# uuwee/Vulkan-PBR-Renderer

Hardware: AMD Instinct MI355X
Metric: IBL-prefilter Mtexels/s (specular prefilter all mips + irradiance; PBR-shaded Mpixels/s under extra.shade_c5 / extra.shade) (higher is better)
Workload: dtype f32; 1 GPU; C4: 4096x4096 specular prefilter (6 faces, 13 mips) + 128x128 irradiance from a 2048^2 HDR cube; env=procedural HDR cube 2048^2 x6 RGBA32F (seed 0x5eed0004, RGBE round-tripped), overlap=False, parallelism=single GPU

## Files before the change

include/gpux.h:

```cpp
#ifndef GPUX_H
#define GPUX_H

#include "gpu_hip.h"

GPU_API void GPUX_SetDevice(int hip_device_index);
GPU_API int  GPUX_GetDevice(void);
typedef void (*GPUX_ErrorHandler)(const char* message, void* user);
GPU_API void GPUX_SetErrorHandler(GPUX_ErrorHandler handler, void* user);
GPU_API const char* GPUX_BackendName(void);

typedef struct GPUX_IBLConstants {
    int32_t mip_level;
    float   roughness;
    float   src_lod;
    int32_t sample_count;
} GPUX_IBLConstants;

GPU_API void GPUX_OpDispatchRows(GPU_Graph* graph, uint32_t face0, uint32_t face1, uint32_t row0, uint32_t row1);
GPU_API void GPUX_OpDispatchLines(GPU_Graph* graph, uint32_t y0, uint32_t y1, uint32_t z0, uint32_t z1);

enum { GPUX_Shade_IBL = 1 << 0, GPUX_Shade_LightShafts = 1 << 1,
       GPUX_Shade_SunShadows = 1 << 2,
       GPUX_Shade_VoxelGI = 1 << 3      };
GPU_API void GPUX_SetShadeFlags(GPU_GraphicsPipeline* pipeline, int flags);
GPU_API void GPUX_OpDrawRows(GPU_Graph* graph, uint32_t row0, uint32_t row1);

GPU_API void GPUX_OpCopyTextureMipToBuffer(GPU_Graph* graph, GPU_Texture* src, uint32_t mip_level, GPU_Buffer* dst, uint32_t dst_offset);
GPU_API void GPUX_OpCopyBufferToTextureMip(GPU_Graph* graph, GPU_Buffer* src, uint32_t src_offset, GPU_Texture* dst, uint32_t mip_level);
GPU_API uint64_t GPUX_TextureMipBytes(const GPU_Texture* texture, uint32_t mip_level);
GPU_API void GPUX_OpCopyDecodedTextureMipToBuffer(GPU_Graph* graph, GPU_Texture* src, uint32_t mip_level, GPU_Buffer* dst, uint32_t dst_offset);
GPU_API void GPUX_OpProjectSH9(GPU_Graph* graph, GPU_Texture* cube, uint32_t mip_level, uint32_t face0, uint32_t face1, uint32_t row0, uint32_t row1,
                               GPU_Buffer* dst, uint32_t dst_offset);
GPU_API void GPUX_OpIrradianceFromSH9(GPU_Graph* graph, GPU_Buffer* src, uint32_t src_offset, GPU_Texture* irradiance_cube, uint32_t mip_level);
GPU_API void* GPUX_TextureDevicePtr(GPU_Texture* texture, uint32_t mip_level);
GPU_API void* GPUX_BufferDevicePtr(GPU_Buffer* buffer);
GPU_API void* GPUX_GraphStream(GPU_Graph* graph);

GPU_API GPU_Texture* GPUX_MakeTextureExternal(GPU_Format format, uint32_t width, uint32_t height, uint32_t depth, GPU_TextureFlags flags,
                                              void* device_memory, uint64_t device_bytes);
GPU_API void GPUX_InvalidateTexture(GPU_Texture* texture);
GPU_API uint64_t GPUX_TextureTotalBytes(const GPU_Texture* texture);
GPU_API uint64_t GPUX_TextureMipOffset(const GPU_Texture* texture, uint32_t mip_level);

GPU_API GPU_Texture* GPUX_MakeCubemapFromEquirect(const void* rgba32f, uint32_t width, uint32_t height, uint32_t face_size, GPU_TextureFlags extra_flags);

GPU_API void GPUX_EnableOpTiming(int enable);
GPU_API uint32_t GPUX_GraphTimedOpCount(GPU_Graph* graph);
GPU_API const char* GPUX_GraphTimedOpName(GPU_Graph* graph, uint32_t index);
GPU_API float GPUX_GraphTimedOpMs(GPU_Graph* graph, uint32_t index);
GPU_API void GPUX_SetPrefilterTolerance(float rel);
GPU_API int GPUX_PrefilterKeptSamples(uint32_t mip_level);
GPU_API float GPUX_GraphSpanMs(GPU_Graph* graph);

GPU_API void GPUX_SetTileStreams(int count);

GPU_API void GPUX_SetGraphReplay(int enable);
GPU_API void GPUX_GraphReplayStats(GPU_Graph* graph, uint64_t* launches, uint64_t* updates, uint64_t* instantiations);
GPU_API uint64_t GPUX_FoldedBlitCount(void);
GPU_API void GPUX_SetGraphOverlap(int on);
GPU_API uint64_t GPUX_OverlappedSubmitCount(void);

GPU_API uint64_t GPUX_RasterRejectedTriangles(void);
GPU_API uint64_t GPUX_VoxelizeFragments(void);

#endif
```

vulkan-pbr-renderer_amd/csrc/gpu_hip.cpp:

```cpp
#include <hip/hip_runtime.h>

#include <math.h>
#include <stdarg.h>
#include <stdio.h>
#include <stdlib.h>
#include <string.h>

#include <map>
#include <string>
#include <vector>

#include "gpux.h"
#include "pbr_kernels.h"

static GPUX_ErrorHandler g_err_handler = nullptr;
static void* g_err_user = nullptr;

static void gpu_fail(const char* fmt, ...) {
    char buf[1024];
    va_list ap;
    va_start(ap, fmt);
    vsnprintf(buf, sizeof buf, fmt, ap);
    va_end(ap);
    if (g_err_handler) { g_err_handler(buf, g_err_user); return; }
    fprintf(stderr, "GPU-ERROR: %s\n", buf);
    fflush(stderr);
    abort();
}
#define GPU_REQUIRE(cond, ret, ...) do { if (!(cond)) { gpu_fail(__VA_ARGS__); return ret; } } while (0)
#define GPU_REQUIRE_V(cond, ...) do { if (!(cond)) { gpu_fail(__VA_ARGS__); return; } } while (0)
#define HIP_OK(call) do { hipError_t e_ = (call); if (e_ != hipSuccess) { gpu_fail("%s: HIP call failed: %s (%s)", __func__, #call, hipGetErrorString(e_)); } } while (0)

enum BindKind { Bind_Texture, Bind_Sampler, Bind_Buffer, Bind_StorageImage };
enum KernelId { Kernel_None = 0, Kernel_BrdfLut, Kernel_Irradiance, Kernel_Prefilter, Kernel_Lighting, Kernel_LightgridSweep, Kernel_TaaResolve, Kernel_FinalPost, Kernel_BloomDown, Kernel_BloomUp, Kernel_SunDepth, Kernel_Geometry, Kernel_Voxelize };

static bool is_bloom_kernel(KernelId k) { return k == Kernel_BloomDown || k == Kernel_BloomUp; }
static bool is_post_kernel(KernelId k) { return is_bloom_kernel(k) || k == Kernel_FinalPost || k == Kernel_TaaResolve; }

struct GPU_Sampler { GPU_SamplerDesc desc; bool shared; };

struct LayoutBinding { std::string name; BindKind kind; GPU_Format format; };
struct GPU_PipelineLayout { std::vector<LayoutBinding> bindings; bool finalized = false; };

struct TextureImpl {
    GPU_Texture base;
    void* dev = nullptr;
    size_t bytes = 0;
    std::vector<size_t> mip_offset;
    uint32_t texel_bytes = 0;
    void* bordered = nullptr;
    size_t bordered_bytes = 0;
    bool bordered_valid = false;
    int bordered_from = 0;
    bool owns_memory = true;
    void* decoded = nullptr; std::vector<size_t> decoded_offset;
    void* cells = nullptr; int cells_first = 0; std::vector<size_t> cells_off; std::vector<char> cells_valid;
    void* lut_cells = nullptr; bool lut_cells_valid = false;
    std::vector<char> range_valid; std::vector<float> range_min, range_max; void* range_dev = nullptr;
};
struct BufferImpl {
// ... 50 lines not shown
    hipEvent_t mid_ev = nullptr;
    bool mid_recorded = false;
    std::vector<TextureImpl*> tail_reads, tail_writes;
    size_t sync_used = 0;
    std::vector<Op> ops;
    bool submitted = false;
    GPU_ComputePipeline* bound_cpipe = nullptr;
    GPU_DescriptorSet* bound_cset = nullptr;
    uint8_t push[128]; uint32_t push_size = 0;
    GPU_RenderPass* preparing = nullptr; GPU_RenderPass* in_pass = nullptr;
    std::vector<DrawParams> draw_params;
    int bound_draw = -1;
    BufferImpl* vertex_buffer = nullptr; BufferImpl* index_buffer = nullptr;
    int raster_op = -1;
    std::vector<RasterScratch> raster; size_t raster_used = 0;
    void* sh_scratch = nullptr; size_t sh_scratch_bytes = 0;
    hipGraphExec_t exec = nullptr;
    bool replay_broken = false;
    uint64_t replay_launches = 0, replay_updates = 0, replay_instantiations = 0;
    std::vector<uint8_t> launch_sig, exec_sig;
    std::vector<hipEvent_t> ev;
    std::vector<std::string> timed_names;
    std::vector<float> timed_ms;
    hipEvent_t span_a = nullptr, span_b = nullptr;
    bool span_recorded = false;
    float span_ms = 0.0f;
};

struct DeviceTable { void* dev = nullptr; int count = 0; float alpha = 0.0f; std::vector<float> weights;  };
struct TableKey {
    int kind, n, aux; uint32_t rbits;
    bool operator<(const TableKey& o) const {
        if (kind != o.kind) return kind < o.kind;
        if (n != o.n) return n < o.n;
        if (aux != o.aux) return aux < o.aux;
        return rbits < o.rbits;
    }
};

static struct {
    GPU_Graph* last_submitted = nullptr;
    bool init = false;
    int device = -1;
    GPU_Sampler samplers[6];
    std::map<TableKey, DeviceTable> tables;
    bool timing = false;
    float prefilter_tol = 0.0f;
    int kept_samples[32] = {0};
    int fold = -1;
    int order = -1;
    int overlap = -1;
    int replay = -1;
    int tile_streams = -1;
    unsigned long long* raster_rejected = nullptr;
    uint64_t raster_rejected_base = 0;
} G;

static const char kTokenLut[] = "HIPK1:gen_brdf_integration_map";
static const char kTokenIrr[] = "HIPK3:gen_irradiance_map";
static const char kTokenPre[] = "HIPK4:gen_prefiltered_env_map";
static const char kTokenLit[] = "HIPK5:lighting_pass";
static const char kTokenSweep[] = "HIPK7:lightgrid_sweep";
static const char kTokenTaa[] = "HIPK8:taa_resolve";
static const char kTokenFinal[] = "HIPK9:final_post_process";
static const char kTokenBloomDown[] = "HIPK10:bloom_downsample";
static const char kTokenBloomUp[] = "HIPK11:bloom_upsample";
static const char kTokenSun[] = "HIPK12:sun_depth_pass";
static const char kTokenGeometry[] = "HIPK13:geometry_pass";
static const char kTokenVoxelize[] = "HIPK14:lightgrid_voxelize";

GPU_API GPU_FormatInfo GPUX_GetFormatInfo(GPU_Format f) {
    struct Row { GPU_Format f; uint32_t ext, size; bool s, v, c, d, st, i; const char* glsl; };
    static const Row rows[] = {
        {GPU_Format_R8UN, 1, 1, 1, 1, 1, 0, 0, 0, "r8"}, {GPU_Format_RG8UN, 1, 2, 1, 1, 1, 0, 0, 0, "rg8"},
        {GPU_Format_RGBA8UN, 1, 4, 1, 1, 1, 0, 0, 0, "rgba8"}, {GPU_Format_BGRA8UN, 1, 4, 1, 1, 1, 0, 0, 0, nullptr},
        {GPU_Format_R16F, 1, 2, 1, 1, 1, 0, 0, 0, "r16f"}, {GPU_Format_RG16F, 1, 4, 1, 1, 1, 0, 0, 0, "rg16f"},
        {GPU_Format_RGB16F, 1, 6, 0, 1, 0, 0, 0, 0, nullptr}, {GPU_Format_RGBA16F, 1, 8, 1, 1, 1, 0, 0, 0, "rgba16f"},
        {GPU_Format_R32F, 1, 4, 1, 1, 1, 0, 0, 0, "r32f"}, {GPU_Format_RG32F, 1, 8, 1, 1, 1, 0, 0, 0, "rg32f"},
        {GPU_Format_RGB32F, 1, 12, 0, 1, 0, 0, 0, 0, nullptr}, {GPU_Format_RGBA32F, 1, 16, 1, 1, 1, 0, 0, 0, "rgba32f"},
        {GPU_Format_R8I, 1, 1, 1, 1, 1, 0, 0, 1, "r8ui"}, {GPU_Format_R16I, 1, 2, 1, 1, 1, 0, 0, 1, "r16ui"},
        {GPU_Format_RG16I, 1, 4, 1, 1, 1, 0, 0, 1, "rg16ui"}, {GPU_Format_RGBA16I, 1, 8, 1, 1, 1, 0, 0, 1, "rgba16ui"},
        {GPU_Format_R32I, 1, 4, 1, 1, 1, 0, 0, 1, "r32ui"}, {GPU_Format_RG32I, 1, 8, 1, 1, 1, 0, 0, 1, "rg32ui"},
        {GPU_Format_RGB32I, 1, 12, 1, 1, 0, 0, 0, 1, nullptr}, {GPU_Format_RGBA32I, 1, 16, 1, 1, 1, 0, 0, 1, "rgba32ui"},
        {GPU_Format_R64I, 1, 8, 0, 0, 0, 0, 0, 1, "r64ui"}, {GPU_Format_D16UN, 1, 2, 1, 0, 0, 1, 0, 0, nullptr},
        {GPU_Format_D32F_Or_X8D24UN, 1, 4, 1, 0, 0, 1, 0, 0, nullptr}, {GPU_Format_D32FS8I_Or_D24UNS8I, 1, 5, 0, 0, 0, 1, 0, 0, nullptr},
        {GPU_Format_D24UNS8I_Or_D32FS8I, 1, 4, 0, 0, 0, 1, 0, 0, nullptr},
        {GPU_Format_BC1_RGB_UN, 4, 8, 1, 0, 0, 0, 0, 0, nullptr}, {GPU_Format_BC1_RGBA_UN, 4, 8, 1, 0, 0, 0, 0, 0, nullptr},
        {GPU_Format_BC3_RGBA_UN, 4, 16, 1, 0, 0, 0, 0, 0, nullptr}, {GPU_Format_BC5_UN, 4, 16, 1, 0, 0, 0, 0, 0, nullptr},
    };
    for (const Row& r : rows)
        if (r.f == f) { GPU_FormatInfo o = {r.ext, r.size, r.s, r.v, r.c, r.d, r.st, r.i, r.glsl}; return o; }
    GPU_FormatInfo z = {0, 0, false, false, false, false, false, false, nullptr};
    return z;
}

GPU_API void GPUX_SetDevice(int idx) { G.device = idx; }
GPU_API int GPUX_GetDevice(void) { return G.device; }
GPU_API void GPUX_SetErrorHandler(GPUX_ErrorHandler h, void* user) { g_err_handler = h; g_err_user = user; }
GPU_API const char* GPUX_BackendName(void) { return "hip-gfx950"; }

static void make_shared_sampler(GPU_Sampler* s, GPU_Filter f, GPU_AddressMode m) {
    memset(&s->desc, 0, sizeof s->desc);
    s->desc.min_filter = s->desc.mag_filter = s->desc.mipmap_mode = f;
    s->desc.address_modes[0] = s->desc.address_modes[1] = s->desc.address_modes[2] = m;
    s->desc.max_lod = 1000.0f;
    s->shared = true;
}

GPU_API void GPU_Init(GPU_WindowHandle window) {
    (void)window;
// ... 1472 lines not shown
    const bool explicit_c = ibl_constants(op, c);
    int n = (explicit_c && c.sample_count > 0) ? c.sample_count : 4096;
    DeviceTable* ang = get_table(2, n, 0.0f, 0);
    DeviceTable* vcs = get_table(3, (int)size, 0.0f, 0);
    if (!ang || !vcs) return;
    int fmt = ot->base.format == GPU_Format_RG16F ? PBRK_FMT_RG16F : (ot->base.format == GPU_Format_RG32F ? PBRK_FMT_RG32F : PBRK_FMT_RGBA32F);
    timed(g, "K1.brdf_lut", ev_used, [&] {
        int rc = pbrk_brdf_lut(out_ptr, fmt, (int)size, n, ang->dev, vcs->dev, (int)op.row0, (int)op.row1, g->cur);
        if (rc != PBRK_OK) gpu_fail("K1 launch failed (%d)", rc);
    });
    ot->bordered_valid = false; ot->lut_cells_valid = false;
}

struct IblPlan {
    bool ok = true;
    bool bad_roughness = false;
    bool copy = false;
    int mip = 0;
    float lod = 0.0f;
    int n = 0;
    float rough = 0.0f, divisor = 1.0f;
    int table_kind = -1;
    DeviceTable* tab = nullptr;
    char name[96];
};
static IblPlan plan_ibl(const Op& op) {
    IblPlan p;
    GPUX_IBLConstants c;
    const bool explicit_c = ibl_constants(op, c);
    p.mip = c.mip_level;
    if (op.cpipe->kernel == Kernel_Irradiance) {
        p.lod = explicit_c ? c.src_lod : 6.0f;
        p.n = (explicit_c && c.sample_count > 0) ? c.sample_count : 1024;
        p.divisor = (float)p.n; p.table_kind = 1;
        snprintf(p.name, sizeof p.name, "K3.irradiance");
    } else if (p.mip == 0) {
        p.copy = true; p.lod = explicit_c ? c.src_lod : 1.0f;
        snprintf(p.name, sizeof p.name, "K4a.prefilter_copy.mip%d", p.mip);
    } else {
        p.lod = explicit_c ? c.src_lod : 3.0f + (float)p.mip;
        p.n = (explicit_c && c.sample_count > 0) ? c.sample_count : 8192;
        p.rough = explicit_c ? c.roughness : reference_roughness(p.mip);
        p.divisor = 3.14159265358979323846f; p.table_kind = 0;
        snprintf(p.name, sizeof p.name, "K4b.prefilter_mc.mip%d", p.mip);
        if (!(p.rough > 0.0f)) { p.bad_roughness = true; p.ok = false; return p; }
    }
    if (p.table_kind >= 0) {
        p.tab = get_table(p.table_kind, p.n, p.rough, 0);
        p.ok = p.tab != nullptr;
    }
    return p;
}

static void exec_ibl_filter(GPU_Graph* g, Op& op, size_t& ev_used) {
    hipStream_t st = g->cur;
    Slot* out = named_slot(op.set, "OUTPUT");
    TextureImpl* ot = out->tex;
    uint32_t size = mip_dim(ot->base.width, out->mip);
    void* out_ptr = (char*)ot->dev + ot->mip_offset[out->mip];
    TextureImpl* et = named_slot(op.set, "TEX_ENV_CUBE")->tex;
    int W = (int)et->base.width, levels = (int)et->base.mip_level_count;
    const IblPlan p = plan_ibl(op);
    if (p.bad_roughness) { gpu_fail("prefilter: roughness must be > 0 for Monte-Carlo mips (got %g)", p.rough); return; }
    if (!p.ok) return;
    const bool mc_prefilter = op.cpipe->kernel == Kernel_Prefilter && !p.copy;
    int l = (int)floorf(p.lod);
    if (l < 0) l = 0;
    if (l > levels - 1) l = levels - 1;
    if ((float)l != p.lod && p.lod < (float)(levels - 1)) { gpu_fail("%s: fractional source LOD %g is not supported by the precompute kernels", p.name, p.lod); return; }
    if (!et->bordered_valid || et->bordered_from > l) {
        timed(g, "apron.env", ev_used, [&] { ensure_bordered(et, st, l); });
        if (!et->bordered_valid || et->bordered_from > l) return;
        publish_side_work(g);
    }
    int n_src = W >> l; if (n_src < 1) n_src = 1;
    const void* src = (const char*)et->bordered + pbrk_bordered_level_offset(W, l) * 16;
    const void* cells = nullptr;
    if (!p.copy) {
        if (cells_ready(et, l)) cells = ensure_cells(et, l, st);
        else { timed(g, "cells.env", ev_used, [&] { cells = ensure_cells(et, l, st); }); publish_side_work(g); }
    }
    int n_keep = p.tab ? p.tab->count : 0;
    if (mc_prefilter && G.prefilter_tol > 0.0f) {
        float mn = 0.0f, mx = 0.0f;
        if (level_range(et, l, st, &mn, &mx)) n_keep = bounded_sample_count(p.tab, mn, mx, G.prefilter_tol);
    }
    if (mc_prefilter && p.mip >= 0 && p.mip < 32) G.kept_samples[p.mip] = n_keep;
    const float alpha = p.table_kind == 0 ? p.tab->alpha : 0.0f;
    timed(g, p.name, ev_used, [&] {
        int rc = p.copy ? pbrk_prefilter_copy(src, n_src, out_ptr, (int)size, (int)op.face0, (int)op.face1, (int)op.row0, (int)op.row1, st)
                        : pbrk_mc_filter(src, cells, n_src, p.tab->dev, n_keep, p.divisor, alpha, out_ptr, (int)size,
                                         (int)op.face0, (int)op.face1, (int)op.row0, (int)op.row1, st);
        if (rc != PBRK_OK) gpu_fail("%s launch failed (%d)", p.name, rc);
    });
    ot->bordered_valid = false;
}

static double dispatch_samples_per_texel(const Op& op) {
    const IblPlan p = plan_ibl(op);
    if (op.cpipe->kernel == Kernel_Irradiance) return p.n;
    if (p.copy) return 4.0;
    return p.tab ? (double)p.tab->count : (double)p.n;
}

static void exec_bloom(GPU_Graph* g, Op& op, size_t& ev_used) {
    GPU_RenderPass* rp = op.pass;
    TextureImpl* target = (TextureImpl*)rp->targets[0].texture;
    TextureImpl* in = named_slot(op.set, "TEX0")->tex;
    PbrkBloomArgs a;
    a.src.data = (char*)in->dev + in->mip_offset[op.mip]; a.src.format = PBRK_FMT_RGBA16F;
    a.src.width = (int)mip_dim(in->base.width, op.mip); a.src.height = (int)mip_dim(in->base.height, op.mip);
    a.dst = (char*)target->dev + target->mip_offset[op.mip2];
    a.dst_width = (int)rp->desc.width; a.dst_height = (int)rp->desc.height;
    int32_t lvl; memcpy(&lvl, op.push, 4); a.dst_mip_level = lvl;
    a.upsample = op.gpipe->kernel == Kernel_BloomUp; a.blend_additive = op.gpipe->blend_additive;
    a.blend_src = op.blend_tex ? (const void*)((const char*)op.blend_tex->dev + op.blend_tex->mip_offset[op.blend_mip]) : nullptr;
    a.y0 = (int)op.row0; a.y1 = (int)op.row1;
    timed(g, a.upsample ? "K11.bloom_upsample" : "K10.bloom_downsample", ev_used, [&] {
        int rc = pbrk_bloom_pass(&a, g->cur);
        if (rc != PBRK_OK) gpu_fail("bloom launch failed (%d)", rc);
    });
}

static void exec_taa(GPU_Graph* g, Op& op, size_t& ev_used) {
    GPU_DescriptorSet* s = op.set;
    GPU_RenderPass* rp = op.pass;
    TextureImpl* target = (TextureImpl*)rp->targets[0].texture;
    PbrkTaaArgs a;
    a.lighting_result = tex2d(named_slot(s, "LIGHTING_RESULT")->tex, PBRK_FMT_RGBA16F);
    a.gbuffer_depth = tex2d(named_slot(s, "GBUFFER_DEPTH")->tex, PBRK_FMT_R32F);
    a.gbuffer_velocity = tex2d(named_slot(s, "GBUFFER_VELOCITY")->tex, PBRK_FMT_RG16F);
    a.gbuffer_velocity_prev = tex2d(named_slot(s, "GBUFFER_VELOCITY_PREV")->tex, PBRK_FMT_RG16F);
    a.prev_frame_result = tex2d(named_slot(s, "PREV_FRAME_RESULT")->tex, PBRK_FMT_RGBA16F);
    a.out = target->dev; a.out_format = out_fmt(target->base.format);
    a.width = (int)rp->desc.width; a.height = (int)rp->desc.height; a.y0 = (int)op.row0; a.y1 = (int)op.row1;
    timed(g, "K8.taa_resolve", ev_used, [&] {
        int rc = pbrk_taa_resolve(&a, g->cur);
        if (rc != PBRK_OK) gpu_fail("K8 launch failed (%d)", rc);
    });
}

static void exec_final(GPU_Graph* g, Op& op, size_t& ev_used) {
    GPU_RenderPass* rp = op.pass;
    TextureImpl* target = (TextureImpl*)rp->targets[0].texture;
    PbrkFinalArgs a;
    a.src = tex2d(named_slot(op.set, "TEX0")->tex, PBRK_FMT_RGBA16F);
    a.out = target->dev; a.out_format = out_fmt(target->base.format);
    a.width = (int)rp->desc.width; a.height = (int)rp->desc.height; a.y0 = (int)op.row0; a.y1 = (int)op.row1;
    timed(g, "K9.final_post_process", ev_used, [&] {
        int rc = pbrk_final_post_process(&a, g->cur);
        if (rc != PBRK_OK) gpu_fail("K9 launch failed (%d)", rc);
    });
}

static void exec_gridview(GPU_Graph* g, Op& op, size_t& ev_used, const float* globals) {
// ... 371 lines not shown
        return true;
    case Op_MipGen: r.push_back(op.tex); w.push_back(op.tex); return true;
    case Op_Blit: r.push_back(op.tex); w.push_back(op.tex2); return true;
    case Op_Clear: w.push_back(op.tex); return true;
    case Op_ProjectSH9: r.push_back(op.tex); return false;
    case Op_IrradianceSH9: w.push_back(op.tex); return false;
    default: return false;
    }
}
static uint64_t g_overlapped_submits = 0;
GPU_API void GPUX_SetGraphOverlap(int on) { G.overlap = on; }
GPU_API uint64_t GPUX_OverlappedSubmitCount(void) { return g_overlapped_submits; }
static bool contains(const std::vector<TextureImpl*>& v, const TextureImpl* t) { for (const TextureImpl* x : v) if (x == t) return true; return false; }

struct OrderPoint {
    GPU_Graph* prev = nullptr;
    size_t before = 0;
};
static OrderPoint order_after_previous(GPU_Graph* g) {
    OrderPoint o;
    GPU_Graph* prev = G.last_submitted;
    G.last_submitted = g;
    if (!env_setting(G.order, "PBR_GRAPH_ORDER", 1) || !prev || prev == g) return o;
    if (!prev->order_ev) HIP_OK(hipEventCreateWithFlags(&prev->order_ev, hipEventDisableTiming));
    HIP_OK(hipEventRecord(prev->order_ev, prev->stream));
    if (overlap_enabled() && prev->mid_recorded && !replay_enabled()) {
        std::vector<TextureImpl*> r, w;
        for (; o.before < g->ops.size(); ++o.before) {
            r.clear(); w.clear();
            if (!op_access(g->ops[o.before], r, w)) break;
            bool clash = false;
            for (TextureImpl* t : w) clash |= contains(prev->tail_reads, t) || contains(prev->tail_writes, t);
            for (TextureImpl* t : r) clash |= contains(prev->tail_writes, t);
            if (clash) break;
        }
    }
    if (o.before > 0) { HIP_OK(hipStreamWaitEvent(g->stream, prev->mid_ev, 0)); o.prev = prev; ++g_overlapped_submits; }
    else HIP_OK(hipStreamWaitEvent(g->stream, prev->order_ev, 0));
    return o;
}

static size_t split_head_tail(GPU_Graph* g, bool overlap_on) {
    size_t mid_idx = g->ops.size();
    for (size_t i = 0; i < g->ops.size(); ++i)
        if (g->ops[i].kind == Op_Shade && is_bloom_kernel(g->ops[i].gpipe->kernel)) { mid_idx = i; break; }
    g->mid_recorded = false; g->tail_reads.clear(); g->tail_writes.clear();
    if (!overlap_on || mid_idx == 0) return g->ops.size();
    bool known = true;
    for (size_t i = mid_idx; i < g->ops.size() && known; ++i) known = op_access(g->ops[i], g->tail_reads, g->tail_writes);
    if (!known) { mid_idx = g->ops.size(); g->tail_reads.clear(); g->tail_writes.clear(); }
    return mid_idx;
}

struct TileRegion {
    struct Wr { TextureImpl* t; uint32_t mip, f0, f1, r0, r1; };
    GPU_Graph* g;
    int n_side;
    std::vector<Wr> writes; std::vector<TextureImpl*> reads;
    bool open = false; size_t rr = 0;

    explicit TileRegion(GPU_Graph* graph) : g(graph) {
        env_setting(G.tile_streams, "PBR_TILE_STREAMS", 4);
        if (G.tile_streams > 16) G.tile_streams = 16;
        n_side = G.tile_streams;
    }
    void close() {
        if (!open) return;
        for (hipStream_t s : g->side) { hipEvent_t e = next_sync_event(g); HIP_OK(hipEventRecord(e, s)); HIP_OK(hipStreamWaitEvent(g->stream, e, 0)); }
        writes.clear(); reads.clear(); open = false; g->cur = g->stream;
    }
    bool wants_side_stream(const Op& op, Slot*& out, Slot*& env) const {
        out = env = nullptr;
        if (!(n_side >= 2 && op.kind == Op_Dispatch && op.rows_explicit && (op.cpipe->kernel == Kernel_Prefilter || op.cpipe->kernel == Kernel_Irradiance))) return false;
        out = named_slot(op.set, "OUTPUT");
        env = named_slot(op.set, "TEX_ENV_CUBE");
        bool tile = true;
        if (out && out->tex) {
            uint32_t size = mip_dim(out->tex->base.width, out->mip);
            double evals = (double)(op.face1 - op.face0) * (op.row1 - op.row0) * size * dispatch_samples_per_texel(op);
            bool whole = op.face0 == 0 && op.face1 == out->tex->base.layer_count && op.row0 == 0 && op.row1 == size;
            if (evals >= (whole ? 1.0e9 : 2.0e6 * 8192.0)) tile = false;
            if (whole && !open) tile = false;
        }
        return tile && out && env && out->tex && env->tex;
    }
    bool place(const Op& op) {
        Slot* out; Slot* env;
        if (!wants_side_stream(op, out, env)) { close(); return false; }
        Wr w = {out->tex, out->mip, op.face0, op.face1, op.row0, op.row1};
        bool clash = w.t == env->tex;
        for (const Wr& o : writes) {
            if (o.t == env->tex) clash = true;
            if (o.t == w.t && o.mip == w.mip && o.f0 < w.f1 && w.f0 < o.f1 && o.r0 < w.r1 && w.r0 < o.r1) clash = true;
        }
        for (TextureImpl* r : reads) if (r == w.t) clash = true;
        if (clash) close();
        if (w.t == env->tex) return false;
        if (!open) {
            while ((int)g->side.size() > n_side) { (void)hipStreamSynchronize(g->side.back()); (void)hipStreamDestroy(g->side.back()); g->side.pop_back(); }
            while ((int)g->side.size() < n_side) { hipStream_t s; HIP_OK(hipStreamCreateWithFlags(&s, hipStreamNonBlocking)); g->side.push_back(s); }
            hipEvent_t e = next_sync_event(g);
            HIP_OK(hipEventRecord(e, g->stream));
            for (hipStream_t s : g->side) HIP_OK(hipStreamWaitEvent(s, e, 0));
            open = true;
        }
        writes.push_back(w); reads.push_back(env->tex);
        g->cur = g->side[rr++ % g->side.size()];
        return true;
    }
};

static bool begin_capture(GPU_Graph* g) {
    if (!replay_enabled() || G.timing || g->replay_broken || g->ops.empty() || !graph_replayable(g)) return false;
    if (hipStreamBeginCapture(g->stream, hipStreamCaptureModeRelaxed) == hipSuccess) return true;
    (void)hipGetLastError(); g->replay_broken = true;
    return false;
}
static void finish_capture(GPU_Graph* g, size_t& ev_used) {
    hipGraph_t cg = nullptr;
    bool ok = hipStreamEndCapture(g->stream, &cg) == hipSuccess && cg;
    if (g->exec && g->exec_sig != g->launch_sig) { (void)hipGraphExecDestroy(g->exec); g->exec = nullptr; }
    if (ok && g->exec) {
        hipGraphNode_t bad = nullptr; hipGraphExecUpdateResult res;
        if (hipGraphExecUpdate(g->exec, cg, &bad, &res) == hipSuccess) ++g->replay_updates;
        else { (void)hipGetLastError(); (void)hipGraphExecDestroy(g->exec); g->exec = nullptr; }
    }
    if (ok && !g->exec) {
        if (hipGraphInstantiate(&g->exec, cg, nullptr, nullptr, 0) == hipSuccess) { ++g->replay_instantiations; g->exec_sig = g->launch_sig; }
        else { (void)hipGetLastError(); g->exec = nullptr; ok = false; }
    }
    if (ok && hipGraphLaunch(g->exec, g->stream) == hipSuccess) ++g->replay_launches; else ok = false;
    if (cg) (void)hipGraphDestroy(cg);
    if (ok) return;
    (void)hipGetLastError();
    g->replay_broken = true;
    if (g->exec) { (void)hipGraphExecDestroy(g->exec); g->exec = nullptr; }
    for (Op& op : g->ops) exec_op(g, op, ev_used);
}

GPU_API void GPU_GraphSubmit(GPU_Graph* g) {
    GPU_REQUIRE_V(g && !g->submitted, "GPU_GraphSubmit: graph is NULL or already submitted");
    GPU_REQUIRE_V(g->in_pass == nullptr && g->preparing == nullptr, "GPU_GraphSubmit: render pass still open");
    if (!snapshot_raster_draws(g)) return;
    g->timed_names.clear(); g->timed_ms.clear();
    size_t ev_used = 0;
    g->sync_used = 0;
    g->launch_sig.clear();
    g->cur = g->stream;
    fold_blits(g);
    OrderPoint order = order_after_previous(g);
    const size_t mid_idx = split_head_tail(g, overlap_enabled());
    if (order.before > mid_idx) order.before = mid_idx;
    g->span_recorded = false;
    if (G.timing) {
        if (!g->span_a) { HIP_OK(hipEventCreate(&g->span_a)); HIP_OK(hipEventCreate(&g->span_b)); }
        HIP_OK(hipEventRecord(g->span_a, g->stream));
    }
    const bool capture = begin_capture(g);
    TileRegion region(g);
    for (size_t i = 0; i < g->ops.size(); ++i) {
        if (order.prev && i == order.before) {
            region.close();
            HIP_OK(hipStreamWaitEvent(g->stream, order.prev->order_ev, 0));
            order.prev = nullptr;
        }
        if (i == mid_idx && !capture) {
            region.close();
            if (!g->mid_ev) HIP_OK(hipEventCreateWithFlags(&g->mid_ev, hipEventDisableTiming));
            HIP_OK(hipEventRecord(g->mid_ev, g->stream));
            g->mid_recorded = true;
        }
        region.place(g->ops[i]);
        exec_op(g, g->ops[i], ev_used);
        g->cur = g->stream;
    }
    region.close();
    if (order.prev) HIP_OK(hipStreamWaitEvent(g->stream, order.prev->order_ev, 0));
    if (G.timing) { HIP_OK(hipEventRecord(g->span_b, g->stream)); g->span_recorded = true; }
    if (capture) finish_capture(g, ev_used);
    g->submitted = true;
}

GPU_API void GPU_GraphWait(GPU_Graph* g) {
    GPU_REQUIRE_V(g, "GPU_GraphWait: NULL graph");
    HIP_OK(hipStreamSynchronize(g->stream));
    g->timed_ms.clear();
    for (size_t i = 0; i < g->timed_names.size(); ++i) {
        float ms = 0.0f;
        HIP_OK(hipEventElapsedTime(&ms, g->ev[2 * i], g->ev[2 * i + 1]));
        g->timed_ms.push_back(ms);
    }
    g->span_ms = 0.0f;
    if (g->span_recorded) { HIP_OK(hipEventElapsedTime(&g->span_ms, g->span_a, g->span_b)); g->span_recorded = false; }
    reset_graph(g);
}

GPU_API void GPUX_EnableOpTiming(int enable) { G.timing = enable != 0; }
GPU_API void GPUX_SetTileStreams(int count) { G.tile_streams = count < 0 ? -1 : count; }
GPU_API uint32_t GPUX_GraphTimedOpCount(GPU_Graph* g) { return g ? (uint32_t)g->timed_ms.size() : 0; }
GPU_API const char* GPUX_GraphTimedOpName(GPU_Graph* g, uint32_t i) { return (g && i < g->timed_names.size()) ? g->timed_names[i].c_str() : ""; }
GPU_API float GPUX_GraphTimedOpMs(GPU_Graph* g, uint32_t i) { return (g && i < g->timed_ms.size()) ? g->timed_ms[i] : 0.0f; }
GPU_API float GPUX_GraphSpanMs(GPU_Graph* g) { return g ? g->span_ms : 0.0f; }
GPU_API void GPUX_SetPrefilterTolerance(float rel) { G.prefilter_tol = rel > 0.0f ? rel : 0.0f; }
GPU_API int GPUX_PrefilterKeptSamples(uint32_t mip) { return mip < 32 ? G.kept_samples[mip] : 0; }
```

vulkan-pbr-renderer_amd/python/pbrhip/__init__.py:

```python
import ctypes as C
import os

import numpy as np

_PKG = os.path.dirname(os.path.abspath(__file__))
PKG_ROOT = os.path.dirname(os.path.dirname(_PKG))
REPO_ROOT = os.path.dirname(PKG_ROOT)
LIB_PATH = os.path.join(PKG_ROOT, "libgpu_hip.so")

(Format_Invalid, Format_R8UN, Format_RG8UN, Format_RGBA8UN, Format_BGRA8UN, Format_R16F, Format_RG16F, Format_RGB16F,
 Format_RGBA16F, Format_R32F, Format_RG32F, Format_RGB32F, Format_RGBA32F, Format_R8I, Format_R16I, Format_RG16I,
 Format_RGBA16I, Format_R32I, Format_RG32I, Format_RGB32I, Format_RGBA32I, Format_R64I, Format_D16UN,
 Format_D32F_Or_X8D24UN) = range(24)
Format_BC1_RGB_UN, Format_BC1_RGBA_UN, Format_BC3_RGBA_UN, Format_BC5_UN = 26, 27, 28, 29
BC_BLOCK_BYTES = {Format_BC1_RGB_UN: 8, Format_BC1_RGBA_UN: 8, Format_BC3_RGBA_UN: 16, Format_BC5_UN: 16}
PBRK_BC1_RGB, PBRK_BC1_RGBA, PBRK_BC3, PBRK_BC5 = 0, 1, 2, 3
PBR_DDS_FILE_MIPS = 1
PBR_DDS_MAX_LEVELS = 16
TextureFlag_StorageImage, TextureFlag_RenderTarget, TextureFlag_HasMipmaps, TextureFlag_Cubemap = 1, 2, 4, 8
BufferFlag_CPU, BufferFlag_GPU, BufferFlag_StorageBuffer = 1, 2, 4
Shade_IBL, Shade_LightShafts = 1, 2
Unit_Prefilter, Unit_Irradiance, Unit_BrdfLut = 0, 1, 2


# ... 131 lines not shown

TexP = C.POINTER(GPU_Texture)
BufP = C.POINTER(GPU_Buffer)
VP = C.c_void_p
U32 = C.c_uint32

PROTOTYPES = {
    "GPU_Init": (None, [VP]), "GPU_Deinit": (None, []), "GPU_WaitUntilIdle": (None, []),
    "GPU_SamplerLinearWrap": (VP, []), "GPU_SamplerLinearClamp": (VP, []), "GPU_SamplerLinearMirror": (VP, []),
    "GPU_SamplerNearestClamp": (VP, []), "GPU_SamplerNearestWrap": (VP, []), "GPU_SamplerNearestMirror": (VP, []),
    "GPU_MakeSampler": (VP, [VP]), "GPU_DestroySampler": (None, [VP]),
    "GPU_InitPipelineLayout": (VP, []), "GPU_TextureBinding": (U32, [VP, C.c_char_p]), "GPU_SamplerBinding": (U32, [VP, C.c_char_p]),
    "GPU_BufferBinding": (U32, [VP, C.c_char_p]), "GPU_StorageImageBinding": (U32, [VP, C.c_char_p, C.c_int]),
    "GPU_FinalizePipelineLayout": (None, [VP]), "GPU_DestroyPipelineLayout": (None, [VP]),
    "GPU_MakeDescriptorArena": (VP, []), "GPU_ResetDescriptorArena": (None, [VP]), "GPU_DestroyDescriptorArena": (None, [VP]),
    "GPU_InitDescriptorSet": (VP, [VP, VP]), "GPU_DestroyDescriptorSet": (None, [VP]),
    "GPU_SetTextureBinding": (None, [VP, U32, TexP]), "GPU_SetTextureMipBinding": (None, [VP, U32, TexP, U32]),
    "GPU_SetSamplerBinding": (None, [VP, U32, VP]), "GPU_SetBufferBinding": (None, [VP, U32, BufP]),
    "GPU_SetStorageImageBinding": (None, [VP, U32, TexP, U32]), "GPU_FinalizeDescriptorSet": (None, [VP]),
    "GPU_MakeTexture": (TexP, [C.c_int, U32, U32, U32, C.c_int, VP]), "GPU_DestroyTexture": (None, [TexP]),
    "GPU_MakeBuffer": (BufP, [U32, C.c_int, VP]), "GPU_DestroyBuffer": (None, [BufP]),
    "GPU_SPIRVFromGLSL": (GPU_String, [VP, C.c_int, VP, C.POINTER(GPU_ShaderDesc), C.POINTER(GPU_GLSLErrorArray)]),
    "GPU_JoinGLSLErrorString": (GPU_String, [VP, GPU_GLSLErrorArray]),
    "GPU_MakeRenderPass": (VP, [VP]), "GPU_DestroyRenderPass": (None, [VP]),
    "GPU_MakeGraphicsPipeline": (VP, [VP]), "GPU_DestroyGraphicsPipeline": (None, [VP]),
    "GPU_MakeComputePipeline": (VP, [VP, C.POINTER(GPU_ShaderDesc)]), "GPU_DestroyComputePipeline": (None, [VP]),
    "GPU_MakeGraph": (VP, []), "GPU_GraphSubmit": (None, [VP]), "GPU_GraphWait": (None, [VP]), "GPU_DestroyGraph": (None, [VP]),
    "GPU_MakeSwapchainGraphs": (None, [U32, C.POINTER(VP)]), "GPU_GetBackbuffer": (TexP, [VP]),
    "GPU_OpBindComputePipeline": (None, [VP, VP]), "GPU_OpBindComputeDescriptorSet": (None, [VP, VP]),
    "GPU_OpPushGraphicsConstants": (None, [VP, VP, VP, U32]), "GPU_OpPushComputeConstants": (None, [VP, VP, VP, U32]),
    "GPU_OpDispatch": (None, [VP, U32, U32, U32]),
    "GPU_OpPrepareRenderPass": (None, [VP, VP]), "GPU_OpPrepareDrawParams": (U32, [VP, VP, VP]),
    "GPU_OpBeginRenderPass": (None, [VP]), "GPU_OpEndRenderPass": (None, [VP]), "GPU_OpBindDrawParams": (None, [VP, U32]),
    "GPU_OpDraw": (None, [VP, U32, U32, U32, U32]), "GPU_OpDrawIndexed": (None, [VP, U32, U32, U32, U32, U32]),
    "GPU_OpBindVertexBuffer": (None, [VP, BufP]), "GPU_OpBindIndexBuffer": (None, [VP, BufP]),
    "GPU_OpCopyBufferToBuffer": (None, [VP, BufP, BufP, U32, U32, U32]),
    "GPU_OpCopyBufferToTexture": (None, [VP, BufP, TexP, U32, U32, U32]), "GPU_OpCopyTextureToBuffer": (None, [VP, TexP, BufP]),
    "GPU_OpBlit": (None, [VP, VP]), "GPU_OpGenerateMipmaps": (None, [VP, TexP]),
    "GPU_OpClearColorF": (None, [VP, TexP, U32, C.c_float, C.c_float, C.c_float, C.c_float]),
    "GPU_OpClearColorI": (None, [VP, TexP, U32, U32, U32, U32, U32]), "GPU_OpClearDepthStencil": (None, [VP, TexP, U32]),
    "GPUX_GetFormatInfo": (None, None),
    "GPUX_SetDevice": (None, [C.c_int]), "GPUX_GetDevice": (C.c_int, []), "GPUX_SetErrorHandler": (None, [VP, VP]),
    "GPUX_BackendName": (C.c_char_p, []), "GPUX_OpDispatchRows": (None, [VP, U32, U32, U32, U32]),
    "GPUX_OpDispatchLines": (None, [VP, U32, U32, U32, U32]),
    "GPUX_SetShadeFlags": (None, [VP, C.c_int]), "GPUX_OpDrawRows": (None, [VP, U32, U32]),
    "GPUX_OpCopyTextureMipToBuffer": (None, [VP, TexP, U32, BufP, U32]), "GPUX_OpCopyBufferToTextureMip": (None, [VP, BufP, U32, TexP, U32]),
    "GPUX_OpCopyDecodedTextureMipToBuffer": (None, [VP, TexP, U32, BufP, U32]),
    "GPUX_FoldedBlitCount": (C.c_uint64, []), "GPUX_SetGraphOverlap": (None, [C.c_int]), "GPUX_OverlappedSubmitCount": (C.c_uint64, []), "GPUX_TextureMipBytes": (C.c_uint64, [TexP, U32]), "GPUX_TextureDevicePtr": (VP, [TexP, U32]), "GPUX_BufferDevicePtr": (VP, [BufP]),
    "GPUX_MakeTextureExternal": (TexP, [C.c_int, U32, U32, U32, C.c_int, VP, C.c_uint64]),
    "GPUX_InvalidateTexture": (None, [TexP]),
    "GPUX_TextureTotalBytes": (C.c_uint64, [TexP]), "GPUX_TextureMipOffset": (C.c_uint64, [TexP, U32]),
    "GPUX_MakeCubemapFromEquirect": (TexP, [VP, U32, U32, U32, C.c_int]),
    "GPUX_RasterRejectedTriangles": (C.c_uint64, []), "GPUX_VoxelizeFragments": (C.c_uint64, []),
    "GPUX_GraphStream": (VP, [VP]), "GPUX_EnableOpTiming": (None, [C.c_int]), "GPUX_SetTileStreams": (None, [C.c_int]), "GPUX_GraphTimedOpCount": (U32, [VP]),
    "GPUX_GraphTimedOpName": (C.c_char_p, [VP, U32]), "GPUX_GraphTimedOpMs": (C.c_float, [VP, U32]), "GPUX_GraphSpanMs": (C.c_float, [VP]),
    "PBR_DecodeHDR": (VP, [VP, C.c_size_t, C.POINTER(C.c_int), C.POINTER(C.c_int), C.POINTER(C.c_char_p)]),
    "PBR_MakeTextureFromHDRIMemory": (TexP, [VP, C.c_size_t]), "PBR_MakeTextureFromHDRIFile": (TexP, [C.c_char_p]),
    "PBR_MakeTextureFromEquirectHDRIMemory": (TexP, [VP, C.c_size_t, U32]), "PBR_MakeTextureFromEquirectHDRIFile": (TexP, [C.c_char_p, U32]),
    "PBR_EncodeHDR": (VP, [VP, C.c_int, C.c_int, C.POINTER(C.c_size_t)]), "PBR_WriteHDRFile": (C.c_int, [C.c_char_p, VP, C.c_int, C.c_int]),
    "PBR_WriteCubeStripHDR": (C.c_int, [C.c_char_p, TexP, U32]),
    "PBR_MakeIBLMaps": (None, [C.POINTER(PBR_IBLMaps), U32, U32, U32]), "PBR_DestroyIBLMaps": (None, [C.POINTER(PBR_IBLMaps)]),
    "PBR_GenIrradianceMap": (None, [TexP, TexP]), "PBR_GenPrefilteredEnvMap": (None, [TexP, TexP, U32]),
    "PBR_GenBRDFIntegrationMap": (None, [TexP]),
    "PBR_MakeIBLPipelines": (VP, []), "PBR_DestroyIBLPipelines": (None, [VP]),
    "PBR_RecordUnits": (None, [VP, VP, VP, TexP, C.POINTER(PBR_IBLMaps), C.POINTER(PBR_WorkUnit), U32]),
    "PBR_PartitionIBL": (U32, [U32, U32, U32, U32, C.c_int, C.c_int, C.POINTER(PBR_WorkUnit), U32]),
    "PBR_ExchangeRanges": (C.c_int, [VP, VP, VP, U32, VP, U32]),
    "PBR_SetRcclLibrary": (C.c_int, [C.c_char_p]), "PBR_RcclInfo": (C.c_int, [C.POINTER(C.c_int), C.POINTER(C.c_char_p)]),
    "PBR_CommInfo": (C.c_int, [VP, C.POINTER(C.c_int), C.POINTER(C.c_int)]),
    "PBR_UnitByteRange": (C.c_int, [C.POINTER(PBR_IBLMaps), C.POINTER(PBR_WorkUnit), C.POINTER(TexP), C.POINTER(C.c_uint64), C.POINTER(C.c_uint64)]),
    "PBR_GatherUnits": (C.c_int64, [VP, VP, C.c_int, C.c_int, C.c_int, C.POINTER(PBR_IBLMaps), U32, U32]),
    "GPUX_SetGraphReplay": (None, [C.c_int]),
    "GPUX_GraphReplayStats": (None, [VP, C.POINTER(C.c_uint64), C.POINTER(C.c_uint64), C.POINTER(C.c_uint64)]),
    "PBR_GatherUnitsMasked": (C.c_int64, [VP, VP, C.c_int, C.c_int, C.c_int, C.POINTER(PBR_IBLMaps), U32, U32, U32]),
    "PBR_GatherPlan": (C.c_int64, [C.c_int, C.c_int, C.c_int, C.POINTER(PBR_IBLMaps), U32, U32, U32, VP, U32]),
    "PBR_SelectUnits": (U32, [C.POINTER(PBR_WorkUnit), U32, U32, C.POINTER(PBR_WorkUnit)]),
    "PBR_RunPartitionedIBL": (C.c_int64, [VP, VP, VP, VP, TexP, C.POINTER(PBR_IBLMaps), VP, C.c_int, C.c_int, C.c_int, U32, U32]),
    "PBR_BandRows": (None, [U32, C.c_int, C.c_int, C.POINTER(U32), C.POINTER(U32)]),
    "PBR_GatherBands": (C.c_int64, [VP, VP, C.c_int, C.c_int, C.c_int, TexP]),
    "PBR_FillGlobals": (None, [C.POINTER(PBR_Globals), C.POINTER(C.c_float), C.POINTER(C.c_float), C.c_float, C.c_float,
                               C.c_float, C.c_float, C.c_float, C.c_float, U32]),
    "PBR_MakeGBuffer": (None, [C.POINTER(PBR_GBuffer), U32, U32, C.c_int]), "PBR_DestroyGBuffer": (None, [C.POINTER(PBR_GBuffer)]),
    "PBR_MakeLightingPass": (VP, [C.POINTER(PBR_GBuffer), C.POINTER(PBR_IBLMaps), U32, U32]), "PBR_DestroyLightingPass": (None, [VP]),
    "PBR_MakeLightingPassEx": (VP, [C.POINTER(PBR_GBuffer), C.POINTER(PBR_IBLMaps), U32, U32, TexP]),
    "PBR_MakeLightingPassLive": (VP, [C.POINTER(PBR_GBuffer), C.POINTER(PBR_IBLMaps), U32, U32, TexP, TexP, TexP]),
    "PBR_LightingGlobalsBuffer": (BufP, [VP]), "PBR_LightingPipeline": (VP, [VP]),
    "PBR_RecordLightingPass": (None, [VP, VP, C.POINTER(PBR_Globals), U32, U32]),
    "PBR_MakePostProcess": (VP, [C.POINTER(PBR_GBuffer), U32, U32, C.c_int]), "PBR_DestroyPostProcess": (None, [VP]),
    "PBR_PostVelocity": (TexP, [VP, U32]), "PBR_PostTaaOutput": (TexP, [VP, U32]), "PBR_PostBackbuffer": (TexP, [VP]),
    "PBR_RecordBloom": (None, [VP, VP, U32]), "PBR_RecordFinalPostProcessBloom": (None, [VP, VP, U32]),
    "PBR_PostBloomDownscale": (TexP, [VP]), "PBR_PostBloomUpscale": (TexP, [VP]), "PBR_PostBloomPassCount": (U32, [VP]),
    "PBR_RecordTaaResolve": (None, [VP, VP, U32]), "PBR_RecordTaaResolveRows": (None, [VP, VP, U32, U32, U32]), "PBR_RecordFinalPostProcess": (None, [VP, VP, U32]),
    "PBR_MakeMesh": (VP, [VP, U32, VP, U32, C.POINTER(PBR_MeshPart), U32]), "PBR_DestroyMesh": (None, [VP]),
    "PBR_MeshVertexBuffer": (BufP, [VP]), "PBR_MeshIndexBuffer": (BufP, [VP]), "PBR_MeshPartCount": (U32, [VP]),
    "PBR_MakeSunDepthPass": (VP, [U32]), "PBR_DestroySunDepthPass": (None, [VP]), "PBR_SunDepthTexture": (TexP, [VP]),
    "PBR_SunDepthGlobalsBuffer": (BufP, [VP]), "PBR_SunDepthPipeline": (VP, [VP]), "PBR_SunDepthRenderPass": (VP, [VP]),
    "PBR_SunDepthLayout": (VP, [VP]), "PBR_SunDepthDescriptorSet": (VP, [VP]),
    "PBR_RecordSunDepthPass": (None, [VP, VP, VP, C.POINTER(PBR_Globals)]),
    "PBR_MakeMaterial": (VP, [U32, VP, VP, VP, VP]), "PBR_DestroyMaterial": (None, [VP]), "PBR_MaterialTexture": (TexP, [VP, U32]),
    "PBR_MeshSetPartMaterial": (None, [VP, U32, VP]),
    "PBR_MakeMaterialFromTextures": (VP, [C.POINTER(TexP)]),
    "PBR_ParseDDS": (C.c_int, [VP, C.c_size_t, C.POINTER(PBR_DDSInfo)]), "PBR_DDSErrorString": (C.c_char_p, [C.c_int]),
    "PBR_MakeTextureFromDDSMemory": (TexP, [VP, C.c_size_t, U32]), "PBR_MakeTextureFromDDSFile": (TexP, [C.c_char_p, U32]),
    "PBR_MakeGeometryPass": (VP, [C.POINTER(PBR_GBuffer), VP, U32, U32]), "PBR_DestroyGeometryPass": (None, [VP]),
    "PBR_GeometryGlobalsBuffer": (BufP, [VP]), "PBR_GeometryPipeline": (VP, [VP, U32]), "PBR_GeometryRenderPass": (VP, [VP, U32]),
    "PBR_GeometryLayout": (VP, [VP]), "PBR_GeometryDescriptorSet": (VP, [VP, VP]),
    "PBR_RecordGeometryPass": (None, [VP, VP, VP, VP, C.POINTER(PBR_Globals), C.POINTER(C.c_float), C.POINTER(C.c_float), U32]),
# ... 313 lines not shown
```

Measured before the change: 2708 Mtexels/s.

## Overlap independent whole-level IBL dispatches across streams with cost-balanced assignment

Detects runs of consecutive whole-level prefilter/irradiance dispatches that write disjoint outputs and do not read each other's outputs. It builds the source aprons and cells for the whole run first, then sorts the dispatches by estimated evaluation count and places each on the least-loaded of a few streams (main plus side streams, two by default). Before this, each whole mip ran serially on the main stream. The goal is to let small mips and the irradiance pass fill idle CUs while a large mip runs. The cost is extra events and stream forks, plus some reordering of the timing records.

```diff
diff --git a/include/gpux.h b/include/gpux.h
--- a/include/gpux.h
+++ b/include/gpux.h
@@ -53,6 +53,9 @@
 GPU_API float GPUX_GraphSpanMs(GPU_Graph* graph);
 
 GPU_API void GPUX_SetTileStreams(int count);
+GPU_API void GPUX_SetLevelOverlap(int on);
+GPU_API void GPUX_SetLevelStreams(int count);
+GPU_API uint32_t GPUX_LevelOverlapCount(void);
 
 GPU_API void GPUX_SetGraphReplay(int enable);
 GPU_API void GPUX_GraphReplayStats(GPU_Graph* graph, uint64_t* launches, uint64_t* updates, uint64_t* instantiations);
diff --git a/vulkan-pbr-renderer_amd/csrc/gpu_hip.cpp b/vulkan-pbr-renderer_amd/csrc/gpu_hip.cpp
--- a/vulkan-pbr-renderer_amd/csrc/gpu_hip.cpp
+++ b/vulkan-pbr-renderer_amd/csrc/gpu_hip.cpp
@@ -6,6 +6,7 @@
 #include <stdlib.h>
 #include <string.h>
 
+#include <algorithm>
 #include <map>
 #include <string>
 #include <vector>
@@ -162,10 +163,13 @@
     int overlap = -1;
     int replay = -1;
     int tile_streams = -1;
+    int level_overlap = 1;
+    int level_streams = -1;
     unsigned long long* raster_rejected = nullptr;
     uint64_t raster_rejected_base = 0;
 } G;
 
+static const int kLevelStreams = 2;
 static const char kTokenLut[] = "HIPK1:gen_brdf_integration_map";
 static const char kTokenIrr[] = "HIPK3:gen_irradiance_map";
 static const char kTokenPre[] = "HIPK4:gen_prefiltered_env_map";
@@ -1744,6 +1748,29 @@
     return p;
 }
 
+static int ibl_source_level(const TextureImpl* et, const IblPlan& p) {
+    const int levels = (int)et->base.mip_level_count;
+    int l = (int)floorf(p.lod);
+    if (l < 0) l = 0;
+    if (l > levels - 1) l = levels - 1;
+    return ((float)l != p.lod && p.lod < (float)(levels - 1)) ? -1 : l;
+}
+
+static bool ensure_ibl_twins(GPU_Graph* g, TextureImpl* et, int l, bool want_cells, size_t& ev_used) {
+    hipStream_t st = g->cur;
+    if (!et->bordered_valid || et->bordered_from > l) {
+        timed(g, "apron.env", ev_used, [&] { ensure_bordered(et, st, l); });
+        if (!et->bordered_valid || et->bordered_from > l) return false;
+        publish_side_work(g);
+    }
+    if (want_cells && !cells_ready(et, l)) {
+        const void* built = nullptr;
+        timed(g, "cells.env", ev_used, [&] { built = ensure_cells(et, l, st); });
+        if (built) publish_side_work(g);
+    }
+    return true;
+}
+
 static void exec_ibl_filter(GPU_Graph* g, Op& op, size_t& ev_used) {
     hipStream_t st = g->cur;
     Slot* out = named_slot(op.set, "OUTPUT");
@@ -1751,27 +1778,17 @@
     uint32_t size = mip_dim(ot->base.width, out->mip);
     void* out_ptr = (char*)ot->dev + ot->mip_offset[out->mip];
     TextureImpl* et = named_slot(op.set, "TEX_ENV_CUBE")->tex;
-    int W = (int)et->base.width, levels = (int)et->base.mip_level_count;
+    int W = (int)et->base.width;
     const IblPlan p = plan_ibl(op);
     if (p.bad_roughness) { gpu_fail("prefilter: roughness must be > 0 for Monte-Carlo mips (got %g)", p.rough); return; }
     if (!p.ok) return;
     const bool mc_prefilter = op.cpipe->kernel == Kernel_Prefilter && !p.copy;
-    int l = (int)floorf(p.lod);
-    if (l < 0) l = 0;
-    if (l > levels - 1) l = levels - 1;
-    if ((float)l != p.lod && p.lod < (float)(levels - 1)) { gpu_fail("%s: fractional source LOD %g is not supported by the precompute kernels", p.name, p.lod); return; }
-    if (!et->bordered_valid || et->bordered_from > l) {
-        timed(g, "apron.env", ev_used, [&] { ensure_bordered(et, st, l); });
-        if (!et->bordered_valid || et->bordered_from > l) return;
-        publish_side_work(g);
-    }
+    const int l = ibl_source_level(et, p);
+    if (l < 0) { gpu_fail("%s: fractional source LOD %g is not supported by the precompute kernels", p.name, p.lod); return; }
+    if (!ensure_ibl_twins(g, et, l, !p.copy, ev_used)) return;
     int n_src = W >> l; if (n_src < 1) n_src = 1;
     const void* src = (const char*)et->bordered + pbrk_bordered_level_offset(W, l) * 16;
-    const void* cells = nullptr;
-    if (!p.copy) {
-        if (cells_ready(et, l)) cells = ensure_cells(et, l, st);
-        else { timed(g, "cells.env", ev_used, [&] { cells = ensure_cells(et, l, st); }); publish_side_work(g); }
-    }
+    const void* cells = p.copy ? nullptr : ensure_cells(et, l, st);
     int n_keep = p.tab ? p.tab->count : 0;
     if (mc_prefilter && G.prefilter_tol > 0.0f) {
         float mn = 0.0f, mx = 0.0f;
@@ -1793,6 +1810,13 @@
     if (op.cpipe->kernel == Kernel_Irradiance) return p.n;
     if (p.copy) return 4.0;
     return p.tab ? (double)p.tab->count : (double)p.n;
+}
+
+static void prepare_ibl_twins(GPU_Graph* g, const Op& op, size_t& ev_used) {
+    TextureImpl* et = named_slot(op.set, "TEX_ENV_CUBE")->tex;
+    const IblPlan p = plan_ibl(op);
+    const int l = p.ok ? ibl_source_level(et, p) : -1;
+    if (l >= 0) ensure_ibl_twins(g, et, l, !p.copy, ev_used);
 }
 
 static void exec_bloom(GPU_Graph* g, Op& op, size_t& ev_used) {
@@ -2270,61 +2294,114 @@
     return mid_idx;
 }
 
+static uint32_t g_level_overlap_count = 0;
 struct TileRegion {
     struct Wr { TextureImpl* t; uint32_t mip, f0, f1, r0, r1; };
     GPU_Graph* g;
-    int n_side;
+    int n_side, n_level;
     std::vector<Wr> writes; std::vector<TextureImpl*> reads;
-    bool open = false; size_t rr = 0;
+    bool open = false; size_t rr = 0, n_open = 0;
 
     explicit TileRegion(GPU_Graph* graph) : g(graph) {
         env_setting(G.tile_streams, "PBR_TILE_STREAMS", 4);
         if (G.tile_streams > 16) G.tile_streams = 16;
         n_side = G.tile_streams;
+        n_level = !G.level_overlap ? 0 : (G.level_streams < 2 ? kLevelStreams : G.level_streams);
+        if (n_level > n_side) n_level = n_side;
+    }
+    void fork(size_t n) {
+        while ((int)g->side.size() > n_side) { (void)hipStreamSynchronize(g->side.back()); (void)hipStreamDestroy(g->side.back()); g->side.pop_back(); }
+        while ((int)g->side.size() < n_side) { hipStream_t s; HIP_OK(hipStreamCreateWithFlags(&s, hipStreamNonBlocking)); g->side.push_back(s); }
+        hipEvent_t e = next_sync_event(g);
+        HIP_OK(hipEventRecord(e, g->stream));
+        for (size_t s = 0; s < n; ++s) HIP_OK(hipStreamWaitEvent(g->side[s], e, 0));
+        open = true; n_open = n;
     }
     void close() {
         if (!open) return;
-        for (hipStream_t s : g->side) { hipEvent_t e = next_sync_event(g); HIP_OK(hipEventRecord(e, s)); HIP_OK(hipStreamWaitEvent(g->stream, e, 0)); }
+        for (size_t s = 0; s < n_open; ++s) { hipEvent_t e = next_sync_event(g); HIP_OK(hipEventRecord(e, g->side[s])); HIP_OK(hipStreamWaitEvent(g->stream, e, 0)); }
         writes.clear(); reads.clear(); open = false; g->cur = g->stream;
     }
-    bool wants_side_stream(const Op& op, Slot*& out, Slot*& env) const {
-        out = env = nullptr;
-        if (!(n_side >= 2 && op.kind == Op_Dispatch && op.rows_explicit && (op.cpipe->kernel == Kernel_Prefilter || op.cpipe->kernel == Kernel_Irradiance))) return false;
+    static bool ibl_dispatch(const Op& op, Slot*& out, Slot*& env, bool& whole) {
+        out = env = nullptr; whole = false;
+        if (!(op.kind == Op_Dispatch && (op.cpipe->kernel == Kernel_Prefilter || op.cpipe->kernel == Kernel_Irradiance))) return false;
         out = named_slot(op.set, "OUTPUT");
         env = named_slot(op.set, "TEX_ENV_CUBE");
-        bool tile = true;
-        if (out && out->tex) {
-            uint32_t size = mip_dim(out->tex->base.width, out->mip);
-            double evals = (double)(op.face1 - op.face0) * (op.row1 - op.row0) * size * dispatch_samples_per_texel(op);
-            bool whole = op.face0 == 0 && op.face1 == out->tex->base.layer_count && op.row0 == 0 && op.row1 == size;
-            if (evals >= (whole ? 1.0e9 : 2.0e6 * 8192.0)) tile = false;
-            if (whole && !open) tile = false;
-        }
-        return tile && out && env && out->tex && env->tex;
-    }
-    bool place(const Op& op) {
-        Slot* out; Slot* env;
-        if (!wants_side_stream(op, out, env)) { close(); return false; }
-        Wr w = {out->tex, out->mip, op.face0, op.face1, op.row0, op.row1};
-        bool clash = w.t == env->tex;
+        if (!(out && env && out->tex && env->tex)) return false;
+        whole = op.face0 == 0 && op.face1 == out->tex->base.layer_count && op.row0 == 0 && op.row1 == mip_dim(out->tex->base.width, out->mip);
+        return true;
+    }
+    static double evaluations(const Op& op, const Slot* out) {
+        return (double)(op.face1 - op.face0) * (op.row1 - op.row0) * mip_dim(out->tex->base.width, out->mip) * dispatch_samples_per_texel(op);
+    }
+    bool clashes(const Wr& w, const TextureImpl* env) const {
+        bool clash = w.t == env;
         for (const Wr& o : writes) {
-            if (o.t == env->tex) clash = true;
+            if (o.t == env) clash = true;
             if (o.t == w.t && o.mip == w.mip && o.f0 < w.f1 && w.f0 < o.f1 && o.r0 < w.r1 && w.r0 < o.r1) clash = true;
         }
         for (TextureImpl* r : reads) if (r == w.t) clash = true;
-        if (clash) close();
-        if (w.t == env->tex) return false;
-        if (!open) {
-            while ((int)g->side.size() > n_side) { (void)hipStreamSynchronize(g->side.back()); (void)hipStreamDestroy(g->side.back()); g->side.pop_back(); }
-            while ((int)g->side.size() < n_side) { hipStream_t s; HIP_OK(hipStreamCreateWithFlags(&s, hipStreamNonBlocking)); g->side.push_back(s); }
-            hipEvent_t e = next_sync_event(g);
-            HIP_OK(hipEventRecord(e, g->stream));
-            for (hipStream_t s : g->side) HIP_OK(hipStreamWaitEvent(s, e, 0));
-            open = true;
-        }
+        return clash;
+    }
+    bool place(const Op& op) {
+        Slot* out; Slot* env; bool whole;
+        bool tile = n_side >= 2 && ibl_dispatch(op, out, env, whole) && (whole ? open : op.rows_explicit && evaluations(op, out) < 2.0e6 * 8192.0);
+        if (!tile) { close(); return false; }
+        Wr w = {out->tex, out->mip, op.face0, op.face1, op.row0, op.row1};
+        if (clashes(w, env->tex)) close();
+        if (w.t == env->tex || (whole && !open)) return false;
+        if (!open) fork((size_t)n_side);
         writes.push_back(w); reads.push_back(env->tex);
         g->cur = g->side[rr++ % g->side.size()];
         return true;
+    }
+    size_t level_run(size_t i, size_t limit) {
+        if (open || n_level < 2) return i;
+        size_t j = i;
+        for (; j < limit; ++j) {
+            const Op& op = g->ops[j];
+            Slot* out; Slot* env; bool whole;
+            if (!ibl_dispatch(op, out, env, whole) || !whole) break;
+            Wr w = {out->tex, out->mip, op.face0, op.face1, op.row0, op.row1};
+            if (clashes(w, env->tex)) break;
+            writes.push_back(w); reads.push_back(env->tex);
+        }
+        writes.clear(); reads.clear();
+        return j - i >= 2 ? j : i;
+    }
+    void run_levels(size_t i, size_t j, size_t& ev_used) {
+        typedef std::pair<size_t, size_t> Range;
+        const size_t base = g->timed_names.size();
+        std::vector<Range> twins(j - i), launch(j - i);
+        std::vector<std::pair<double, size_t>> by_cost;
+        for (size_t k = i; k < j; ++k) {
+            Slot* out; Slot* env; bool whole;
+            ibl_dispatch(g->ops[k], out, env, whole);
+            twins[k - i].first = g->timed_names.size();
+            prepare_ibl_twins(g, g->ops[k], ev_used);
+            twins[k - i].second = g->timed_names.size();
+            by_cost.push_back({evaluations(g->ops[k], out), k});
+        }
+        std::stable_sort(by_cost.begin(), by_cost.end(), [](const std::pair<double, size_t>& a, const std::pair<double, size_t>& b) { return a.first > b.first; });
+        std::vector<double> load(std::min((size_t)n_level, j - i), 0.0);
+        fork(load.size() - 1);
+        for (const std::pair<double, size_t>& c : by_cost) {
+            const size_t s = (size_t)(std::min_element(load.begin(), load.end()) - load.begin());
+            load[s] += c.first;
+            g->cur = s ? g->side[s - 1] : g->stream;
+            launch[c.second - i].first = g->timed_names.size();
+            exec_op(g, g->ops[c.second], ev_used);
+            launch[c.second - i].second = g->timed_names.size();
+        }
+        g_level_overlap_count += (uint32_t)(j - i);
+        close();
+        if (g->timed_names.size() == base) return;
+        std::vector<std::string> names; std::vector<hipEvent_t> evs;
+        for (size_t k = 0; k < j - i; ++k)
+            for (const Range& r : {twins[k], launch[k]})
+                for (size_t e = r.first; e < r.second; ++e) { names.push_back(g->timed_names[e]); evs.push_back(g->ev[2 * e]); evs.push_back(g->ev[2 * e + 1]); }
+        std::copy(names.begin(), names.end(), g->timed_names.begin() + (ptrdiff_t)base);
+        std::copy(evs.begin(), evs.end(), g->ev.begin() + (ptrdiff_t)(2 * base));
     }
 };
 
@@ -2376,6 +2453,7 @@
     }
     const bool capture = begin_capture(g);
     TileRegion region(g);
+    g_level_overlap_count = 0;
     for (size_t i = 0; i < g->ops.size(); ++i) {
         if (order.prev && i == order.before) {
             region.close();
@@ -2388,6 +2466,8 @@
             HIP_OK(hipEventRecord(g->mid_ev, g->stream));
             g->mid_recorded = true;
         }
+        const size_t run_end = region.level_run(i, order.prev && i < order.before ? order.before : g->ops.size());
+        if (run_end > i) { region.run_levels(i, run_end, ev_used); i = run_end - 1; continue; }
         region.place(g->ops[i]);
         exec_op(g, g->ops[i], ev_used);
         g->cur = g->stream;
@@ -2415,6 +2495,9 @@
 
 GPU_API void GPUX_EnableOpTiming(int enable) { G.timing = enable != 0; }
 GPU_API void GPUX_SetTileStreams(int count) { G.tile_streams = count < 0 ? -1 : count; }
+GPU_API void GPUX_SetLevelOverlap(int on) { G.level_overlap = on != 0; }
+GPU_API void GPUX_SetLevelStreams(int count) { G.level_streams = count < 2 ? -1 : count; }
+GPU_API uint32_t GPUX_LevelOverlapCount(void) { return g_level_overlap_count; }
 GPU_API uint32_t GPUX_GraphTimedOpCount(GPU_Graph* g) { return g ? (uint32_t)g->timed_ms.size() : 0; }
 GPU_API const char* GPUX_GraphTimedOpName(GPU_Graph* g, uint32_t i) { return (g && i < g->timed_names.size()) ? g->timed_names[i].c_str() : ""; }
 GPU_API float GPUX_GraphTimedOpMs(GPU_Graph* g, uint32_t i) { return (g && i < g->timed_ms.size()) ? g->timed_ms[i] : 0.0f; }
diff --git a/vulkan-pbr-renderer_amd/python/pbrhip/__init__.py b/vulkan-pbr-renderer_amd/python/pbrhip/__init__.py
--- a/vulkan-pbr-renderer_amd/python/pbrhip/__init__.py
+++ b/vulkan-pbr-renderer_amd/python/pbrhip/__init__.py
@@ -207,7 +207,7 @@
     "GPUX_TextureTotalBytes": (C.c_uint64, [TexP]), "GPUX_TextureMipOffset": (C.c_uint64, [TexP, U32]),
     "GPUX_MakeCubemapFromEquirect": (TexP, [VP, U32, U32, U32, C.c_int]),
     "GPUX_RasterRejectedTriangles": (C.c_uint64, []), "GPUX_VoxelizeFragments": (C.c_uint64, []),
-    "GPUX_GraphStream": (VP, [VP]), "GPUX_EnableOpTiming": (None, [C.c_int]), "GPUX_SetTileStreams": (None, [C.c_int]), "GPUX_GraphTimedOpCount": (U32, [VP]),
+    "GPUX_GraphStream": (VP, [VP]), "GPUX_EnableOpTiming": (None, [C.c_int]), "GPUX_SetTileStreams": (None, [C.c_int]), "GPUX_SetLevelOverlap": (None, [C.c_int]), "GPUX_SetLevelStreams": (None, [C.c_int]), "GPUX_LevelOverlapCount": (U32, []), "GPUX_GraphTimedOpCount": (U32, [VP]),
     "GPUX_GraphTimedOpName": (C.c_char_p, [VP, U32]), "GPUX_GraphTimedOpMs": (C.c_float, [VP, U32]), "GPUX_GraphSpanMs": (C.c_float, [VP]),
     "PBR_DecodeHDR": (VP, [VP, C.c_size_t, C.POINTER(C.c_int), C.POINTER(C.c_int), C.POINTER(C.c_char_p)]),
     "PBR_MakeTextureFromHDRIMemory": (TexP, [VP, C.c_size_t]), "PBR_MakeTextureFromHDRIFile": (TexP, [C.c_char_p]),
```

Result: faster. 2796 Mtexels/s (median of 6 runs) (+3.3%).
